# apcamargo/genomad

Measured on NVIDIA H100. Metric: nn_classification_windows_per_s, higher is better.
Workload: dtype split operands on wgmma (conv: fp16 main pass + two e4m3 correction passes; w_v: 3 fp16 passes), fp32 accumulate; fp32-equivalent (<=1e-4 vs the fp32 oracle, measured ~1e-5)

## Files before the change

### genomad_b200/csrc/api.cu

```cuda
#include <cuda.h>
#include <cuda_runtime.h>
#include <cuda_fp16.h>

#include <algorithm>
#include <cmath>
#include <cstdio>
#include <cstring>
#include <string>
#include <vector>

#include "../../include/gnm.h"
#include "common.cuh"
#include "encode.cuh"
#include "conv_t.cuh"
#include "layer1_wv.cuh"
#include "conv_ref.cuh"
#include "igloo.cuh"
#include "dense.cuh"
#include "logits_tc.cuh"
#include "wv_gather.cuh"

using namespace gnm;

static thread_local std::string g_err;
static int fail(const std::string& m) { g_err = m; return 1; }

#define GNM_CUDA(expr)                                                                       \
  do {                                                                                       \
    cudaError_t e__ = (expr);                                                                \
    if (e__ != cudaSuccess)                                                                  \
      return fail(std::string(#expr) + " failed: " + cudaGetErrorString(e__) + " (" __FILE__ \
                  ":" + std::to_string(__LINE__) + ")");                                     \
  } while (0)

extern "C" const char* gnm_last_error(void) { return g_err.c_str(); }
extern "C" const char* gnm_version(void) { return "libgnm 0.4 (sm_90a; wgmma fp16 + e4m3 split convs, fused fp16x3 w_v + patch gather, tf32x3 logits and dense head)"; }

struct StageTimer {
  std::vector<const char*> names;
  std::vector<cudaEvent_t> events;
};

struct gnm_handle {
  int device = 0;
  int max_batch = 0;
  int num_sms = 0;
  long long launches = 0;
  int conv_impl = 0;
  int debug_stop = 0;
  int profile_stages = 0;
  int conv_experiment = 0;
  int conv_cluster = 1;
  int fuse_gather = 1;
  int fuse_l1 = 0;
  long long* conv_dbg = nullptr;
  float* conv1_table = nullptr; float* conv1_triple = nullptr; float* conv1_bias = nullptr;
  uint8_t* wpack[4] = {nullptr, nullptr, nullptr, nullptr};
  float conv_out_scale[2] = {1.f, 1.f};
  float* conv_bias[2] = {nullptr, nullptr};
  float* conv_w32[2] = {nullptr, nullptr};
  float* wv32[2] = {nullptr, nullptr};
  float* ent_w[2] = {nullptr, nullptr}; int32_t* ent_pos[2] = {nullptr, nullptr}; int32_t* slot_of[2] = {nullptr, nullptr};
  float* wbias[2] = {nullptr, nullptr}; float* wqk[2] = {nullptr, nullptr};
  float* d0w = nullptr; float* d0b = nullptr; float* bn0_scale = nullptr; float* bn0_shift = nullptr;
  float* d1w = nullptr; float* d1b = nullptr; float* bn1_scale = nullptr; float* bn1_shift = nullptr;
  float* d2w = nullptr; float* d2b = nullptr;
  float* dwT_hi[2] = {nullptr, nullptr}; float* dwT_lo[2] = {nullptr, nullptr};
  float* hA_hi[2] = {nullptr, nullptr}; float* hA_lo[2] = {nullptr, nullptr};
  CUtensorMap tm_hd_a[2][2]; CUtensorMap tm_hd_b[2][2];
  uint8_t* ybuf[2] = {nullptr, nullptr};
  int ybuf_fp8lo[2] = {0, 0};
  float* q[2] = {nullptr, nullptr};
  float* mpi[2] = {nullptr, nullptr};
  float* mpi_hi[2] = {nullptr, nullptr}; float* mpi_lo[2] = {nullptr, nullptr};
  float* wqkT_hi[2] = {nullptr, nullptr}; float* wqkT_lo[2] = {nullptr, nullptr};
  CUtensorMap tm_lg_a[2][2];
  CUtensorMap tm_lg_b[2][2];
  float* part = nullptr;
  int2* grp[2] = {nullptr, nullptr};
  int32_t* band_gstart[2] = {nullptr, nullptr};
  uint4* wfrag[2] = {nullptr, nullptr};
  float gather_unscale[2] = {1.f, 1.f};
  float wv_out_scale[2] = {1.f, 1.f};
  std::vector<int32_t> band_groups[2];
  int32_t* cta_split = nullptr;
  std::vector<int32_t> split_host[2];
  int split_groups[2] = {-1, -1}, split_grid[2] = {-1, -1};
  float wv_cost_base = 1.f, wv_cost_group = 0.1f;
  int mb_pad = 0;
  CUtensorMap tm_band[2];
  float* logits = nullptr; float* logits_part = nullptr; float* h0 = nullptr; float* h1 = nullptr; float* h2 = nullptr;
  float* scratch32 = nullptr;
  uint8_t* in_stage[2] = {nullptr, nullptr};
  float* out_stage[2] = {nullptr, nullptr};
  float* q_set[2][2] = {{nullptr, nullptr}, {nullptr, nullptr}};
  float* mpi_set[2][2] = {{nullptr, nullptr}, {nullptr, nullptr}};
  float* mpi_hi_set[2][2] = {{nullptr, nullptr}, {nullptr, nullptr}};
  float* mpi_lo_set[2][2] = {{nullptr, nullptr}, {nullptr, nullptr}};
  CUtensorMap tm_lg_a_set[2][2][2];
  int tail_overlap = 1;
  cudaStream_t tail_stream = nullptr;
  cudaEvent_t main_done[2] = {nullptr, nullptr}, tail_done[2] = {nullptr, nullptr};
  cudaStream_t copy_stream = nullptr, compute_stream = nullptr;
  cudaEvent_t in_ready[2] = {nullptr, nullptr}, in_free[2] = {nullptr, nullptr};
  DeviceStatus* status = nullptr;
  CUtensorMap tm_act[2];
  CUtensorMap tm_w[4];
  CUtensorMap tm_w_half[4];
  StageTimer timer;
  std::vector<void*> allocs;
};

template <class T>
static int dev_upload(gnm_handle* h, T** dst, const T* src, size_t count) {
  GNM_CUDA(cudaMalloc(reinterpret_cast<void**>(dst), count * sizeof(T)));
  h->allocs.push_back(*dst);
  GNM_CUDA(cudaMemcpy(*dst, src, count * sizeof(T), cudaMemcpyHostToDevice));
  return 0;
}
template <class T>
static int dev_alloc(gnm_handle* h, T** dst, size_t count) {
  GNM_CUDA(cudaMalloc(reinterpret_cast<void**>(dst), count * sizeof(T)));
  h->allocs.push_back(*dst);
  return 0;
}

typedef CUresult (*PFN_encodeTiled)(CUtensorMap*, CUtensorMapDataType, cuuint32_t, void*, const cuuint64_t*,
                                    const cuuint64_t*, const cuuint32_t*, const cuuint32_t*, CUtensorMapInterleave,
                                    CUtensorMapSwizzle, CUtensorMapL2promotion, CUtensorMapFloatOOBfill);

static int get_encode_fn(PFN_encodeTiled* fn) {
  void* p = nullptr;
  cudaDriverEntryPointQueryResult qres;
  GNM_CUDA(cudaGetDriverEntryPoint("cuTensorMapEncodeTiled", &p, cudaEnableDefault, &qres));
  if (qres != cudaDriverEntryPointSuccess || !p) return fail("cuTensorMapEncodeTiled not available from the driver");
  *fn = reinterpret_cast<PFN_encodeTiled>(p);
  return 0;
}

static int make_act_map(PFN_encodeTiled enc, CUtensorMap* tm, uint8_t* base, int n_windows, int box_rows = kSlabRows) {
  cuuint64_t dims[3] = {kRowBytes, kTok, static_cast<cuuint64_t>(n_windows)};
  cuuint64_t strides[2] = {kRowBytes, static_cast<cuuint64_t>(kTok) * kRowBytes};
  cuuint32_t box[3] = {128, static_cast<cuuint32_t>(box_rows), 1};
  cuuint32_t estr[3] = {1, 1, 1};
  CUresult r = enc(tm, CU_TENSOR_MAP_DATA_TYPE_UINT8, 3, base, dims, strides, box, estr,
                   CU_TENSOR_MAP_INTERLEAVE_NONE, CU_TENSOR_MAP_SWIZZLE_128B, CU_TENSOR_MAP_L2_PROMOTION_L2_128B,
                   CU_TENSOR_MAP_FLOAT_OOB_FILL_NONE);
  if (r != CUDA_SUCCESS) return fail("cuTensorMapEncodeTiled(activations) failed: " + std::to_string(int(r)));
  return 0;
}
static int make_band_map(PFN_encodeTiled enc, CUtensorMap* tm, uint8_t* base, int n_windows) {
  cuuint64_t dims[3] = {kRowBytes, static_cast<cuuint64_t>(n_windows), kTok};
  cuuint64_t strides[2] = {static_cast<cuuint64_t>(kTok) * kRowBytes, kRowBytes};
  cuuint32_t box[3] = {128, kBandWins, kBandRows};
  cuuint32_t estr[3] = {1, 1, 1};
  CUresult r = enc(tm, CU_TENSOR_MAP_DATA_TYPE_UINT8, 3, base, dims, strides, box, estr,
                   CU_TENSOR_MAP_INTERLEAVE_NONE, CU_TENSOR_MAP_SWIZZLE_128B, CU_TENSOR_MAP_L2_PROMOTION_L2_128B,
                   CU_TENSOR_MAP_FLOAT_OOB_FILL_NONE);
  if (r != CUDA_SUCCESS) return fail("cuTensorMapEncodeTiled(activation bands) failed: " + std::to_string(int(r)));
  return 0;
}
static int make_w_map(PFN_encodeTiled enc, CUtensorMap* tm, uint8_t* base, int n_stages, int box_rows) {
  cuuint64_t dims[2] = {128, static_cast<cuuint64_t>(n_stages) * 128};
  cuuint64_t strides[1] = {128};
  cuuint32_t box[2] = {128, static_cast<cuuint32_t>(box_rows)};
  cuuint32_t estr[2] = {1, 1};
  CUresult r = enc(tm, CU_TENSOR_MAP_DATA_TYPE_UINT8, 2, base, dims, strides, box, estr,
                   CU_TENSOR_MAP_INTERLEAVE_NONE, CU_TENSOR_MAP_SWIZZLE_128B, CU_TENSOR_MAP_L2_PROMOTION_L2_256B,
                   CU_TENSOR_MAP_FLOAT_OOB_FILL_NONE);
  if (r != CUDA_SUCCESS) return fail("cuTensorMapEncodeTiled(weights) failed: " + std::to_string(int(r)));
  return 0;
}

static int make_f32_map(PFN_encodeTiled enc, CUtensorMap* tm, float* base, int inner, int rows, int box_rows) {
  cuuint64_t dims[2] = {static_cast<cuuint64_t>(inner), static_cast<cuuint64_t>(rows)};
  cuuint64_t strides[1] = {static_cast<cuuint64_t>(inner) * sizeof(float)};
  cuuint32_t box[2] = {32, static_cast<cuuint32_t>(box_rows)};
  cuuint32_t estr[2] = {1, 1};
  CUresult r = enc(tm, CU_TENSOR_MAP_DATA_TYPE_FLOAT32, 2, base, dims, strides, box, estr,
                   CU_TENSOR_MAP_INTERLEAVE_NONE, CU_TENSOR_MAP_SWIZZLE_128B, CU_TENSOR_MAP_L2_PROMOTION_L2_256B,
                   CU_TENSOR_MAP_FLOAT_OOB_FILL_NONE);
  if (r != CUDA_SUCCESS) return fail("cuTensorMapEncodeTiled(fp32 matrix) failed: " + std::to_string(int(r)));
  return 0;
}

static void pack_stage_f16(std::vector<uint8_t>& dst, const float* Wkn , int w_lo, int kh, float scale) {
  for (int n = 0; n < kC; ++n)
    for (int kk = 0; kk < 64; ++kk) {
      const float x = Wkn[static_cast<size_t>(kh * 64 + kk) * kC + n] * scale;
      const __half hi = __float2half_rn(x);
      const float v = w_lo ? x - __half2float(hi) : __half2float(hi);
      const uint16_t bits = __half_as_ushort(__float2half_rn(v));
      dst.push_back(static_cast<uint8_t>(bits & 0xff));
      dst.push_back(static_cast<uint8_t>(bits >> 8));
    }
}
static void pack_stage_f8_pairs(std::vector<uint8_t>& dst, const float* Wkn, int kh, float scale, float scale_hi, float scale_lo) {
  for (int n = 0; n < kC; ++n)
    for (int c = 0; c < 64; ++c) {
      const float x = Wkn[static_cast<size_t>(kh * 64 + c) * kC + n] * scale;
      const float hi = __half2float(__float2half_rn(x));
      dst.push_back(static_cast<uint8_t>(__nv_cvt_float_to_fp8(hi * scale_hi, __NV_SATFINITE, __NV_E4M3)));
      dst.push_back(static_cast<uint8_t>(__nv_cvt_float_to_fp8((x - hi) * scale_lo, __NV_SATFINITE, __NV_E4M3)));
    }
}

struct PatchPack {
  std::vector<float> ent_w;
  std::vector<int32_t> ent_pos, slot_of;
  std::vector<int2> groups;
  std::vector<int32_t> band_gstart;
  std::vector<uint32_t> frag;
  float unscale = 1.f;
};
static void pack_patches(const int32_t* patches, const float* w_mult, const float* w_summer, PatchPack& o) {
  std::vector<int> order(static_cast<size_t>(kPatches) * kPatchLen);
  for (size_t i = 0; i < order.size(); ++i) order[i] = static_cast<int>(i);
  std::stable_sort(order.begin(), order.end(), [&](int a, int b) { return patches[a] < patches[b]; });
  o.ent_w.assign(static_cast<size_t>(kGsSlots) * kC, 0.f);
  o.ent_pos.assign(kGsSlots, 0);
  o.slot_of.assign(static_cast<size_t>(kPatches) * kPatchLen, 0);
  std::vector<float>& ent_w = o.ent_w;
  std::vector<int32_t>& ent_pos = o.ent_pos;
  for (size_t slot = 0; slot < order.size(); ++slot) {
    const int e = order[slot], k = e % kPatchLen;
    ent_pos[slot] = patches[e];
    o.slot_of[e] = static_cast<int32_t>(slot);
    for (int c = 0; c < kC; ++c)
      ent_w[slot * kC + c] = (w_mult[static_cast<size_t>(e) * kC + c] * w_summer[k * kC + c]) * (1.f / kActScale);
  }
  float wmax = 0.f;
  for (float v : ent_w) wmax = std::max(wmax, std::fabs(v));
  int k2 = 0;
  if (wmax > 0.f && std::isfinite(wmax)) { int ex; std::frexp(wmax, &ex); k2 = std::max(-24, std::min(40, 14 - ex)); }
  const float wscale = std::ldexp(1.f, k2);
  o.unscale = std::ldexp(1.f, -k2);
  o.groups.clear();
  o.band_gstart.assign(kNumBands + 1, 0);
  const size_t n_ent = order.size();
  size_t slot = 0;
  for (int b = 0; b < kNumBands; ++b) {
    o.band_gstart[b] = static_cast<int32_t>(o.groups.size());
    while (slot < n_ent && ent_pos[slot] < (b + 1) * kBandRows) {
      size_t run = slot;
      while (run < n_ent && ent_pos[run] == ent_pos[slot] && run - slot < static_cast<size_t>(kWgGroupMax)) ++run;
      o.groups.push_back(make_int2(static_cast<int>(slot), (ent_pos[slot] - b * kBandRows) | (static_cast<int>(run - slot) << 8)));
      slot = run;
    }
  }
  o.band_gstart[kNumBands] = static_cast<int32_t>(o.groups.size());
  if (o.groups.empty()) o.groups.push_back(make_int2(0, 0));
  auto h2 = [](float x, float y) {
    return static_cast<uint32_t>(__half_as_ushort(__float2half_rn(x))) | (static_cast<uint32_t>(__half_as_ushort(__float2half_rn(y))) << 16);
  };
  o.frag.assign(static_cast<size_t>(kGsSlots) * 128, 0u);
  for (size_t e = 0; e < n_ent; ++e)
    for (int kh = 0; kh < 2; ++kh)
      for (int ks = 0; ks < 4; ++ks)
        for (int tig = 0; tig < 4; ++tig) {
          const int k0 = kh * 64 + ks * 16 + 2 * tig;
          const int kk[4] = {k0, k0 + 1, k0 + 8, k0 + 9};
          float hi[4], lo[4];
          for (int i = 0; i < 4; ++i) {
            const float x = ent_w[e * kC + kk[i]] * wscale;
            hi[i] = __half2float(__float2half_rn(x));
            lo[i] = x - hi[i];
          }
          uint32_t* f = &o.frag[(((e * 2 + kh) * 4 + ks) * 4 + tig) * 4];
          f[0] = h2(hi[0], hi[1]); f[1] = h2(hi[2], hi[3]); f[2] = h2(lo[0], lo[1]); f[3] = h2(lo[2], lo[3]);
        }
}
extern "C" int gnm_pack_patches(const int32_t* patches, const float* w_mult, const float* w_summer, int32_t* slot_of, int32_t* ent_pos,
                                float* ent_w, int32_t* groups, int* n_groups, int32_t* band_first_group, uint32_t* frag, float* unscale,
                                int* layout) {
  if (layout) { layout[0] = kBandRows; layout[1] = kNumBands; layout[2] = kGsSlots; layout[3] = kWgGroupMax; }
  if (!patches && !w_mult && !w_summer) return 0;
  if (!patches || !w_mult || !w_summer || !n_groups) return fail("gnm_pack_patches: null argument");
  for (int i = 0; i < kPatches * kPatchLen; ++i)
    if (patches[i] < 0 || patches[i] >= kTok) return fail("gnm_pack_patches: patch index out of range");
  PatchPack pk;
  pack_patches(patches, w_mult, w_summer, pk);
  const int real_groups = pk.band_gstart[kNumBands];
  if (groups && *n_groups < real_groups) return fail("gnm_pack_patches: groups buffer too small");
  if (slot_of) std::memcpy(slot_of, pk.slot_of.data(), pk.slot_of.size() * sizeof(int32_t));
  if (ent_pos) std::memcpy(ent_pos, pk.ent_pos.data(), pk.ent_pos.size() * sizeof(int32_t));
  if (ent_w) std::memcpy(ent_w, pk.ent_w.data(), pk.ent_w.size() * sizeof(float));
  if (groups) for (int i = 0; i < real_groups; ++i) { groups[2 * i] = pk.groups[i].x; groups[2 * i + 1] = pk.groups[i].y; }
  *n_groups = real_groups;
  if (band_first_group) std::memcpy(band_first_group, pk.band_gstart.data(), pk.band_gstart.size() * sizeof(int32_t));
  if (frag) std::memcpy(frag, pk.frag.data(), pk.frag.size() * sizeof(uint32_t));
  if (unscale) *unscale = pk.unscale;
  return 0;
}

extern "C" int gnm_create(int device, const gnm_weights* w, int max_batch, gnm_handle** out) {
  if (!w || !out) return fail("gnm_create: null argument");
  if (max_batch < 1 || max_batch > 32768) return fail("gnm_create: max_batch must be in [1, 32768]");
  int ndev = 0;
  if (cudaGetDeviceCount(&ndev) != cudaSuccess || ndev == 0)
    return fail("gnm_create: no CUDA device available (libgnm has no CPU fallback)");
  if (device < 0 || device >= ndev) return fail("gnm_create: bad device index");
  cudaDeviceProp prop;
  GNM_CUDA(cudaGetDeviceProperties(&prop, device));
  if (prop.major != 9 || prop.minor != 0)
    return fail(std::string("gnm_create: device is sm_") + std::to_string(prop.major * 10 + prop.minor) +
                ", this library is built for sm_90a (H100) only");
  GNM_CUDA(cudaSetDevice(device));
// ... 764 lines not shown
```

### genomad_b200/csrc/wv_gather.cuh

```cuda
#pragma once
#include <cuda.h>
#include <type_traits>
#include "common.cuh"
#include "conv_t.cuh"
#include "igloo.cuh"

namespace gnm {

constexpr int kBandRows   = 24;
constexpr int kBandWins   = 8;
constexpr int kWgN        = kBandRows * kBandWins;
constexpr int kNumBands   = (kTok + kBandRows - 1) / kBandRows;
constexpr int kWgRegion   = kWgN * 128;
constexpr int kWgBufs     = 6;
constexpr int kWgSlab     = kWgBufs * kWgRegion;
constexpr int kWgWBytes   = kWvStages * kBStage;
constexpr int kWgMmaWarps = 8;
constexpr int kWgWarps    = 15;
constexpr int kWgThreads  = (kWgMmaWarps + kWgWarps + 1) * 32;
constexpr int kWgGroupCap = 2;
constexpr int kWgGroupMax = 4;
constexpr int kWgSmem     = kWgSlab + kWgWBytes + 2048;
static_assert(kWgSmem <= 232448, "wv_gather_kernel exceeds the 227 KB of shared memory a CTA may use");
static_assert(kWgN == 3 * 64 && kBandRows == 3 * kPool && kBandWins == 8, "unit shape: three pool groups of 8 positions x 8 windows");
static_assert(kWgRegion % 1024 == 0, "regions must keep the 1024-byte alignment of the 128-byte swizzle");

struct WvGatherParams {
  float* q_out;
  float out_scale;
  const int2* grp;
  const int32_t* band_gstart;
  const uint4* wfrag;
  float gather_unscale;
  float* part_t;
  int n_windows, n_pad;
  int groups;
  int n_units;
  const int32_t* cta_split;
  int experiment;
  long long* dbg;
  DeviceStatus* status;
};

__device__ __forceinline__ uint2 ldg_frag(const uint2* p) {
  uint2 v;
  asm volatile("ld.global.nc.L1::evict_last.v2.u32 {%0, %1}, [%2];" : "=r"(v.x), "=r"(v.y) : "l"(p));
  return v;
}
__device__ __forceinline__ void ldsm_x4(uint32_t saddr, uint32_t (&a)[4]) {
  asm volatile("ldmatrix.sync.aligned.m8n8.x4.shared.b16 {%0, %1, %2, %3}, [%4];"
               : "=r"(a[0]), "=r"(a[1]), "=r"(a[2]), "=r"(a[3]) : "r"(saddr));
}
__device__ __forceinline__ void mma_16816(float (&d)[4], const uint32_t (&a)[4], uint32_t b0, uint32_t b1) {
  asm volatile("mma.sync.aligned.m16n8k16.row.col.f32.f16.f16.f32 {%0, %1, %2, %3}, {%4, %5, %6, %7}, {%8, %9}, {%0, %1, %2, %3};"
               : "+f"(d[0]), "+f"(d[1]), "+f"(d[2]), "+f"(d[3]) : "r"(a[0]), "r"(a[1]), "r"(a[2]), "r"(a[3]), "r"(b0), "r"(b1));
}

__global__ void __launch_bounds__(kWgThreads, 1)
wv_gather_kernel(const __grid_constant__ CUtensorMap tm_band, const __grid_constant__ CUtensorMap tm_w, const WvGatherParams p) {
  extern __shared__ uint8_t smem_raw[];
  uint8_t* smem = reinterpret_cast<uint8_t*>((reinterpret_cast<uintptr_t>(smem_raw) + 1023) & ~uintptr_t(1023));
  uint8_t* s_a = smem;
  uint8_t* s_w = smem + kWgSlab;
  uint64_t* bars = reinterpret_cast<uint64_t*>(s_w + kWgWBytes);
  uint64_t* a_full = bars;
  uint64_t* a_empty = bars + 8;
  uint64_t* w_full = bars + 16;

  const int warp = threadIdx.x >> 5, lane = threadIdx.x & 31;
  constexpr int kProducerWarp = kWgMmaWarps + kWgWarps;
  const int u_begin = p.cta_split[blockIdx.x], u_end = p.cta_split[blockIdx.x + 1];

  if (warp == kProducerWarp && lane == 0) {
    tma_prefetch_desc(&tm_band);
    tma_prefetch_desc(&tm_w);
    for (int i = 0; i < kWgBufs; ++i) { mbar_init(&a_full[i], 1); mbar_init(&a_empty[i], kWgMmaWarps + kWgWarps); }
    mbar_init(w_full, 1);
    fence_barrier_init();
  }
  __syncthreads();

  if (warp == kProducerWarp && lane == 0) {
    mbar_arrive_expect_tx(w_full, kWgWBytes);
    for (int q = 0; q < kWvStages; ++q) tma_load_2d_hint(s_w + q * kBStage, &tm_w, w_full, 0, q * 128, l2_policy_evict_last());
    const uint64_t pol = l2_policy_evict_first();
    uint32_t phases = 0;
    int b0 = 0;
    for (int unit = u_begin; unit < u_end; ++unit) {
      const int band = unit / p.groups;
      const int w0 = (unit - band * p.groups) * kBandWins;
#pragma unroll
      for (int k = 0; k < 4; ++k) {
        int b = b0 + k; if (b >= kWgBufs) b -= kWgBufs;
        mbar_wait(&a_empty[b], ((phases >> b) & 1) ^ 1, p.status, 500 + b);
        phases ^= 1u << b;
        mbar_arrive_expect_tx(&a_full[b], kWgRegion);
        const int src = (k & 1 ? kOffLo16 : kOffHi16) + (k >> 1) * 128;
        tma_load_3d_hint(s_a + b * kWgRegion, &tm_band, &a_full[b], src, w0, band * kBandRows, pol);
      }
      b0 += 4; if (b0 >= kWgBufs) b0 -= kWgBufs;
    }
  } else if (warp < kWgMmaWarps) {
    const int g = warp >> 2, wq = warp & 3;
    const uint32_t a_base = smem_u32(s_a);
    const uint32_t w_base = smem_u32(s_w) + g * 64 * 128;
    const int ch0 = g * 64 + wq * 16 + (lane >> 2);
    const int win0 = 2 * (lane & 3);
    const float oscale = p.out_scale;
    mbar_wait(w_full, 0, p.status, 510);
    uint32_t phases = 0;
    int b0 = 0;
    float d[32];
    for (int unit = u_begin; unit < u_end; ++unit) {
      const int band = unit / p.groups;
      const int w0 = (unit - band * p.groups) * kBandWins;
      int bufs[4];
#pragma unroll
      for (int k = 0; k < 4; ++k) {
        int b = b0 + k; if (b >= kWgBufs) b -= kWgBufs;
        bufs[k] = b;
        mbar_wait(&a_full[b], (phases >> b) & 1, p.status, 530 + b);
        phases ^= 1u << b;
      }
#pragma unroll 1
      for (int pg = 0; pg < kBandRows / kPool; ++pg) {
        wgmma_fence();
#pragma unroll 1
        for (int kh = 0; kh < 2; ++kh) {
          const uint64_t yh = gmma_desc_sw128(a_base + bufs[2 * kh] * kWgRegion + pg * 64 * 128);
          const uint64_t yl = gmma_desc_sw128(a_base + bufs[2 * kh + 1] * kWgRegion + pg * 64 * 128);
          const uint64_t whi = gmma_desc_sw128(w_base + (2 * kh) * kBStage);
          const uint64_t wlo = gmma_desc_sw128(w_base + (2 * kh + 1) * kBStage);
#pragma unroll
          for (int kk = 0; kk < 4; ++kk) {
            wgmma_f16_n64(d, whi + kk * 2, yh + kk * 2, (kh == 0 && kk == 0) ? 0u : 1u);
            wgmma_f16_n64(d, whi + kk * 2, yl + kk * 2, 1u);
          }
#pragma unroll
          for (int kk = 0; kk < 4; ++kk) wgmma_f16_n64(d, wlo + kk * 2, yh + kk * 2, 1u);
        }
        wgmma_commit();
        wgmma_wait<0>();
        wgmma_fence_regs(d);
        const int gg = band * (kBandRows / kPool) + pg;
        if (gg < kPooled && !(p.experiment & 128)) {
#pragma unroll
          for (int h = 0; h < 2; ++h)
#pragma unroll
            for (int e = 0; e < 2; ++e) {
              float m = d[2 * h + e];
#pragma unroll
              for (int i = 1; i < kPool; ++i) m = fmaxf(m, d[4 * i + 2 * h + e]);
              const int w = w0 + win0 + e;
              if (w < p.n_windows) p.q_out[(static_cast<size_t>(w) * kPooled + gg) * kC + ch0 + 8 * h] = m * oscale;
            }
        }
      }
      __syncwarp();
      if (lane == 0)
#pragma unroll
        for (int k = 0; k < 4; ++k) mbar_arrive(&a_empty[bufs[k]]);
      b0 += 4; if (b0 >= kWgBufs) b0 -= kWgBufs;
    }
  } else if (warp >= kWgMmaWarps && warp < kWgMmaWarps + kWgWarps) {
    const int gw = warp - kWgMmaWarps;
    const float gscale = p.gather_unscale;
    const int lm_plane = (lane >> 3) & 1, lm_chunk = lane >> 4, lm_win = lane & 7;
    const int gid = lane >> 2, tig = lane & 3;
    const uint32_t slab = smem_u32(s_a);
    int it = 0;
    uint32_t phases = 0;
    int b0 = 0;
    long long c_wait_full = 0, c_gather = 0, tq = 0;
    const long long t_begin = clock64();
    int cur_band = -1, g_first = 0, g_cnt = 0, n_mine = 0;
    int my_e0[kWgGroupCap] = {0, 0}, my_meta[kWgGroupCap] = {0, 0};
    bool fast = true;
    auto gather_group = [&](int e0, int meta, int kh, uint32_t hi_base, uint32_t lo_base) -> float {
      const int row = meta & 31, ne = meta >> 8;
      const uint2* wf = reinterpret_cast<const uint2*>(p.wfrag) + ((static_cast<size_t>(e0 + (gid >> 1)) * 2 + kh) * 16 + tig) * 2 + (gid & 1);
      uint2 b[4];
#pragma unroll
      for (int ks = 0; ks < 4; ++ks) b[ks] = ((gid >> 1) < ne && !(p.experiment & 1024)) ? ldg_frag(wf + ks * 8) : make_uint2(0u, 0u);
      const uint32_t rb = (lm_plane ? lo_base : hi_base) + row * (kBandWins * 128) + lm_win * 128;
      uint32_t a[4][4];
#pragma unroll
      for (int ks = 0; ks < 4; ++ks) {
        if (p.experiment & 2048) { a[ks][0] = a[ks][1] = a[ks][2] = a[ks][3] = rb; continue; }
        ldsm_x4(rb + (((ks * 2 + lm_chunk) ^ lm_win) << 4), a[ks]);
      }
      float d[4][4];
#pragma unroll
      for (int ks = 0; ks < 4; ++ks) d[ks][0] = d[ks][1] = d[ks][2] = d[ks][3] = 0.f;
      if (p.experiment & 256) {
#pragma unroll
        for (int ks = 0; ks < 4; ++ks) asm volatile("" :: "r"(a[ks][0] | a[ks][1] | a[ks][2] | a[ks][3] | b[ks].x | b[ks].y));
      } else {
#pragma unroll
        for (int ks = 0; ks < 4; ++ks) mma_16816(d[ks], a[ks], b[ks].x, b[ks].y);
      }
      float v = 0.f;
#pragma unroll
      for (int ks = 0; ks < 4; ++ks) v += (d[ks][0] + d[ks][2]) + (d[ks][1] + d[ks][3]);
      return v * gscale;
    };
    for (int unit = u_begin; unit < u_end; ++unit, ++it) {
      const int band = unit / p.groups;
      const int w0 = (unit - band * p.groups) * kBandWins;
      if (band != cur_band) {
        cur_band = band;
        g_first = p.band_gstart[band];
        g_cnt = (p.experiment & 32) ? 0 : p.band_gstart[band + 1] - g_first;
        fast = g_cnt <= kWgWarps * kWgGroupCap;
        n_mine = 0;
#pragma unroll
        for (int i = 0; i < kWgGroupCap; ++i) {
          const int gi = gw + i * kWgWarps;
          if (fast && gi < g_cnt) { const int2 m = p.grp[g_first + gi]; my_e0[i] = m.x; my_meta[i] = m.y; n_mine = i + 1; }
        }
      }
      float c0[kWgGroupCap];
#pragma unroll 1
      for (int kh = 0; kh < 2; ++kh) {
        int bh = b0 + 2 * kh; if (bh >= kWgBufs) bh -= kWgBufs;
        int bl = b0 + 2 * kh + 1; if (bl >= kWgBufs) bl -= kWgBufs;
        const uint32_t ph_h = (phases >> bh) & 1, ph_l = (phases >> bl) & 1;
        phases ^= (1u << bh) | (1u << bl);
        const uint32_t hi_base = slab + bh * kWgRegion, lo_base = slab + bl * kWgRegion;
        if (p.dbg) tq = clock64();
        mbar_wait(&a_full[bh], ph_h, p.status, 550 + bh);
        mbar_wait(&a_full[bl], ph_l, p.status, 560 + bl);
        if (p.dbg) { const long long t = clock64(); c_wait_full += t - tq; tq = t; }
        if (fast) {
#pragma unroll
          for (int i = 0; i < kWgGroupCap; ++i)
            if (i < n_mine) {
              const float v = gather_group(my_e0[i], my_meta[i], kh, hi_base, lo_base);
              if (kh == 0) c0[i] = v;
              else if (tig < (my_meta[i] >> 8) && !(p.experiment & 64))
                p.part_t[static_cast<size_t>(my_e0[i] + tig) * p.n_pad + w0 + gid] = c0[i] + v;
            }
        } else {
#pragma unroll 1
          for (int gi = gw; gi < g_cnt; gi += kWgWarps) {
            const int2 m = p.grp[g_first + gi];
            const float v = gather_group(m.x, m.y, kh, hi_base, lo_base);
            if (tig < (m.y >> 8)) {
              float* gp = p.part_t + static_cast<size_t>(m.x + tig) * p.n_pad + w0 + gid;
              *gp = kh == 0 ? v : *gp + v;
            }
          }
        }
        __syncwarp();
        if (lane == 0) { mbar_arrive(&a_empty[bh]); mbar_arrive(&a_empty[bl]); }
        if (p.dbg) c_gather += clock64() - tq;
      }
      b0 += 4; if (b0 >= kWgBufs) b0 -= kWgBufs;
    }
    if (p.dbg && warp == kWgMmaWarps && lane == 0) {
      long long* d = p.dbg + blockIdx.x * 8;
      d[0] = clock64() - t_begin; d[1] = c_wait_full; d[2] = c_gather; d[5] = it;
    }
  }
}

__global__ void __launch_bounds__(256)
patch_finish_t_kernel(const float* __restrict__ part_t, const int32_t* __restrict__ slot_of, const float* __restrict__ w_bias,
                      float* __restrict__ mpi, float* __restrict__ mpi_hi, float* __restrict__ mpi_lo, int n_windows, int n_pad) {
  __shared__ float tile[32][33];
  const int p0 = blockIdx.x * 32, w0 = blockIdx.y * 32;
  const int tx = threadIdx.x & 31, ty = threadIdx.x >> 5;
  for (int pp = ty; pp < 32; pp += 8) {
    const int pch = p0 + pp, w = w0 + tx;
    float v = 0.f;
    if (pch < kPatches && w < n_windows) {
      const int4 s4 = *reinterpret_cast<const int4*>(slot_of + pch * 4);
      v = (((part_t[static_cast<size_t>(s4.x) * n_pad + w] + part_t[static_cast<size_t>(s4.y) * n_pad + w]) +
            part_t[static_cast<size_t>(s4.z) * n_pad + w]) + part_t[static_cast<size_t>(s4.w) * n_pad + w]) + w_bias[pch];
    }
    tile[pp][tx] = v;
  }
  __syncthreads();
  for (int ww = ty; ww < 32; ww += 8) {
    const int pch = p0 + tx, w = w0 + ww;
    if (pch < kPatches && w < n_windows) {
      const float v = tile[tx][ww];
      const size_t o = static_cast<size_t>(w) * kPatches + pch;
      mpi[o] = v;
      const float hi = __uint_as_float(__float_as_uint(v) & 0xffffe000u);
      mpi_hi[o] = hi;
      mpi_lo[o] = __uint_as_float(__float_as_uint(v - hi) & 0xffffe000u);
    }
  }
}

}
```

Before: 74440.

## Pipeline w_v gather at pool-group granularity with an 18-slot TMA box ring

Replaces the six band-sized shared buffers with an 18-slot ring of smaller boxes, one box per pool group, plane and half. The producer now issues four boxes per pool group, and consumers release slots after each pool group instead of after a whole band. The goal is to shorten the pipeline stall between units and keep the wgmma and gather warps fed with a deeper prefetch. Gather warps now process both k-halves of a group together and skip groups outside the current pool group. The cost is more TMA issues and barrier traffic, plus always-on clock64 timing in the MMA warps.

```diff
diff --git a/genomad_b200/csrc/api.cu b/genomad_b200/csrc/api.cu
--- a/genomad_b200/csrc/api.cu
+++ b/genomad_b200/csrc/api.cu
@@ -152,7 +152,7 @@
 static int make_band_map(PFN_encodeTiled enc, CUtensorMap* tm, uint8_t* base, int n_windows) {
   cuuint64_t dims[3] = {kRowBytes, static_cast<cuuint64_t>(n_windows), kTok};
   cuuint64_t strides[2] = {static_cast<cuuint64_t>(kTok) * kRowBytes, kRowBytes};
-  cuuint32_t box[3] = {128, kBandWins, kBandRows};
+  cuuint32_t box[3] = {128, kBandWins, kPool};
   cuuint32_t estr[3] = {1, 1, 1};
   CUresult r = enc(tm, CU_TENSOR_MAP_DATA_TYPE_UINT8, 3, base, dims, strides, box, estr,
                    CU_TENSOR_MAP_INTERLEAVE_NONE, CU_TENSOR_MAP_SWIZZLE_128B, CU_TENSOR_MAP_L2_PROMOTION_L2_128B,
diff --git a/genomad_b200/csrc/wv_gather.cuh b/genomad_b200/csrc/wv_gather.cuh
--- a/genomad_b200/csrc/wv_gather.cuh
+++ b/genomad_b200/csrc/wv_gather.cuh
@@ -11,9 +11,10 @@
 constexpr int kBandWins   = 8;
 constexpr int kWgN        = kBandRows * kBandWins;
 constexpr int kNumBands   = (kTok + kBandRows - 1) / kBandRows;
-constexpr int kWgRegion   = kWgN * 128;
-constexpr int kWgBufs     = 6;
-constexpr int kWgSlab     = kWgBufs * kWgRegion;
+constexpr int kWgBox      = kPool * kBandWins * 128;
+constexpr int kWgBoxes    = 4 * (kBandRows / kPool);
+constexpr int kWgSlots    = 18;
+constexpr int kWgSlab     = kWgSlots * kWgBox;
 constexpr int kWgWBytes   = kWvStages * kBStage;
 constexpr int kWgMmaWarps = 8;
 constexpr int kWgWarps    = 15;
@@ -23,7 +24,8 @@
 constexpr int kWgSmem     = kWgSlab + kWgWBytes + 2048;
 static_assert(kWgSmem <= 232448, "wv_gather_kernel exceeds the 227 KB of shared memory a CTA may use");
 static_assert(kWgN == 3 * 64 && kBandRows == 3 * kPool && kBandWins == 8, "unit shape: three pool groups of 8 positions x 8 windows");
-static_assert(kWgRegion % 1024 == 0, "regions must keep the 1024-byte alignment of the 128-byte swizzle");
+static_assert(kWgBox % 1024 == 0, "boxes must keep the 1024-byte alignment of the 128-byte swizzle");
+static_assert(kWgSlots >= 4, "every consumer holds one pool group's four boxes at a time");
 
 struct WvGatherParams {
   float* q_out;
@@ -56,6 +58,9 @@
                : "+f"(d[0]), "+f"(d[1]), "+f"(d[2]), "+f"(d[3]) : "r"(a[0]), "r"(a[1]), "r"(a[2]), "r"(a[3]), "r"(b0), "r"(b1));
 }
 
+__device__ __forceinline__ uint32_t wg_slot(uint32_t L) { return L % kWgSlots; }
+__device__ __forceinline__ uint32_t wg_parity(uint32_t L) { return (L / kWgSlots) & 1; }
+
 __global__ void __launch_bounds__(kWgThreads, 1)
 wv_gather_kernel(const __grid_constant__ CUtensorMap tm_band, const __grid_constant__ CUtensorMap tm_w, const WvGatherParams p) {
   extern __shared__ uint8_t smem_raw[];
@@ -64,41 +69,44 @@
   uint8_t* s_w = smem + kWgSlab;
   uint64_t* bars = reinterpret_cast<uint64_t*>(s_w + kWgWBytes);
   uint64_t* a_full = bars;
-  uint64_t* a_empty = bars + 8;
-  uint64_t* w_full = bars + 16;
-
-  const int warp = threadIdx.x >> 5, lane = threadIdx.x & 31;
+  uint64_t* a_empty = bars + kWgSlots;
+  uint64_t* w_full = bars + 2 * kWgSlots;
+
+  const int warp = __shfl_sync(0xffffffffu, static_cast<int>(threadIdx.x) >> 5, 0);
+  const int lane = threadIdx.x & 31;
   constexpr int kProducerWarp = kWgMmaWarps + kWgWarps;
   const int u_begin = p.cta_split[blockIdx.x], u_end = p.cta_split[blockIdx.x + 1];
 
-  if (warp == kProducerWarp && lane == 0) {
-    tma_prefetch_desc(&tm_band);
-    tma_prefetch_desc(&tm_w);
-    for (int i = 0; i < kWgBufs; ++i) { mbar_init(&a_full[i], 1); mbar_init(&a_empty[i], kWgMmaWarps + kWgWarps); }
-    mbar_init(w_full, 1);
-    fence_barrier_init();
+  if (warp == kProducerWarp) {
+    if (elect_one()) {
+      tma_prefetch_desc(&tm_band);
+      tma_prefetch_desc(&tm_w);
+      for (int i = 0; i < kWgSlots; ++i) { mbar_init(&a_full[i], 1); mbar_init(&a_empty[i], kWgMmaWarps + kWgWarps); }
+      mbar_init(w_full, 1);
+      fence_barrier_init();
+    }
   }
   __syncthreads();
 
-  if (warp == kProducerWarp && lane == 0) {
-    mbar_arrive_expect_tx(w_full, kWgWBytes);
-    for (int q = 0; q < kWvStages; ++q) tma_load_2d_hint(s_w + q * kBStage, &tm_w, w_full, 0, q * 128, l2_policy_evict_last());
-    const uint64_t pol = l2_policy_evict_first();
-    uint32_t phases = 0;
-    int b0 = 0;
-    for (int unit = u_begin; unit < u_end; ++unit) {
-      const int band = unit / p.groups;
-      const int w0 = (unit - band * p.groups) * kBandWins;
-#pragma unroll
-      for (int k = 0; k < 4; ++k) {
-        int b = b0 + k; if (b >= kWgBufs) b -= kWgBufs;
-        mbar_wait(&a_empty[b], ((phases >> b) & 1) ^ 1, p.status, 500 + b);
-        phases ^= 1u << b;
-        mbar_arrive_expect_tx(&a_full[b], kWgRegion);
-        const int src = (k & 1 ? kOffLo16 : kOffHi16) + (k >> 1) * 128;
-        tma_load_3d_hint(s_a + b * kWgRegion, &tm_band, &a_full[b], src, w0, band * kBandRows, pol);
-      }
-      b0 += 4; if (b0 >= kWgBufs) b0 -= kWgBufs;
+  if (warp == kProducerWarp) {
+    if (elect_one()) {
+      mbar_arrive_expect_tx(w_full, kWgWBytes);
+      for (int q = 0; q < kWvStages; ++q) tma_load_2d_hint(s_w + q * kBStage, &tm_w, w_full, 0, q * 128, l2_policy_evict_last());
+      const uint64_t pol = l2_policy_evict_first();
+      uint32_t L = 0;
+      for (int unit = u_begin; unit < u_end; ++unit) {
+        const int band = unit / p.groups;
+        const int w0 = (unit - band * p.groups) * kBandWins;
+        for (int pg = 0; pg < kBandRows / kPool; ++pg)
+#pragma unroll
+          for (int r = 0; r < 4; ++r, ++L) {
+            const uint32_t s = wg_slot(L);
+            mbar_wait(&a_empty[s], wg_parity(L) ^ 1, p.status, 500 + s);
+            mbar_arrive_expect_tx(&a_full[s], kWgBox);
+            const int src = (r & 1 ? kOffLo16 : kOffHi16) + (r >> 1) * 128;
+            tma_load_3d_hint(s_a + s * kWgBox, &tm_band, &a_full[s], src, w0, band * kBandRows + pg * kPool, pol);
+          }
+      }
     }
   } else if (warp < kWgMmaWarps) {
     const int g = warp >> 2, wq = warp & 3;
@@ -108,27 +116,28 @@
     const int win0 = 2 * (lane & 3);
     const float oscale = p.out_scale;
     mbar_wait(w_full, 0, p.status, 510);
-    uint32_t phases = 0;
-    int b0 = 0;
+    long long c_wait = 0, c_mma = 0, c_epi = 0;
+    uint32_t L = 0;
     float d[32];
     for (int unit = u_begin; unit < u_end; ++unit) {
       const int band = unit / p.groups;
       const int w0 = (unit - band * p.groups) * kBandWins;
-      int bufs[4];
-#pragma unroll
-      for (int k = 0; k < 4; ++k) {
-        int b = b0 + k; if (b >= kWgBufs) b -= kWgBufs;
-        bufs[k] = b;
-        mbar_wait(&a_full[b], (phases >> b) & 1, p.status, 530 + b);
-        phases ^= 1u << b;
-      }
 #pragma unroll 1
-      for (int pg = 0; pg < kBandRows / kPool; ++pg) {
+      for (int pg = 0; pg < kBandRows / kPool; ++pg, L += 4) {
+        uint32_t s[4];
+        long long tq = clock64();
+#pragma unroll
+        for (int r = 0; r < 4; ++r) {
+          s[r] = wg_slot(L + r);
+          mbar_wait(&a_full[s[r]], wg_parity(L + r), p.status, 530 + r);
+        }
+        long long t = clock64();
+        c_wait += t - tq; tq = t;
         wgmma_fence();
-#pragma unroll 1
+#pragma unroll
         for (int kh = 0; kh < 2; ++kh) {
-          const uint64_t yh = gmma_desc_sw128(a_base + bufs[2 * kh] * kWgRegion + pg * 64 * 128);
-          const uint64_t yl = gmma_desc_sw128(a_base + bufs[2 * kh + 1] * kWgRegion + pg * 64 * 128);
+          const uint64_t yh = gmma_desc_sw128(a_base + s[2 * kh] * kWgBox);
+          const uint64_t yl = gmma_desc_sw128(a_base + s[2 * kh + 1] * kWgBox);
           const uint64_t whi = gmma_desc_sw128(w_base + (2 * kh) * kBStage);
           const uint64_t wlo = gmma_desc_sw128(w_base + (2 * kh + 1) * kBStage);
 #pragma unroll
@@ -142,6 +151,12 @@
         wgmma_commit();
         wgmma_wait<0>();
         wgmma_fence_regs(d);
+        t = clock64();
+        c_mma += t - tq; tq = t;
+        __syncwarp();
+        if (lane == 0)
+#pragma unroll
+          for (int r = 0; r < 4; ++r) mbar_arrive(&a_empty[s[r]]);
         const int gg = band * (kBandRows / kPool) + pg;
         if (gg < kPooled && !(p.experiment & 128)) {
 #pragma unroll
@@ -155,34 +170,33 @@
               if (w < p.n_windows) p.q_out[(static_cast<size_t>(w) * kPooled + gg) * kC + ch0 + 8 * h] = m * oscale;
             }
         }
-      }
-      __syncwarp();
-      if (lane == 0)
-#pragma unroll
-        for (int k = 0; k < 4; ++k) mbar_arrive(&a_empty[bufs[k]]);
-      b0 += 4; if (b0 >= kWgBufs) b0 -= kWgBufs;
-    }
-  } else if (warp >= kWgMmaWarps && warp < kWgMmaWarps + kWgWarps) {
+        c_epi += clock64() - tq;
+      }
+    }
+    if (p.dbg && wq == 0 && lane == 0) {
+      long long* dd = p.dbg + blockIdx.x * 8;
+      if (g == 0) { dd[3] = c_wait; dd[4] = c_mma; dd[6] = c_epi; }
+      else dd[7] = c_mma;
+    }
+  } else {
     const int gw = warp - kWgMmaWarps;
     const float gscale = p.gather_unscale;
     const int lm_plane = (lane >> 3) & 1, lm_chunk = lane >> 4, lm_win = lane & 7;
     const int gid = lane >> 2, tig = lane & 3;
     const uint32_t slab = smem_u32(s_a);
     int it = 0;
-    uint32_t phases = 0;
-    int b0 = 0;
     long long c_wait_full = 0, c_gather = 0, tq = 0;
     const long long t_begin = clock64();
     int cur_band = -1, g_first = 0, g_cnt = 0, n_mine = 0;
     int my_e0[kWgGroupCap] = {0, 0}, my_meta[kWgGroupCap] = {0, 0};
     bool fast = true;
-    auto gather_group = [&](int e0, int meta, int kh, uint32_t hi_base, uint32_t lo_base) -> float {
+    auto gather_group = [&](int e0, int meta, int kh, uint32_t Lp) -> float {
       const int row = meta & 31, ne = meta >> 8;
       const uint2* wf = reinterpret_cast<const uint2*>(p.wfrag) + ((static_cast<size_t>(e0 + (gid >> 1)) * 2 + kh) * 16 + tig) * 2 + (gid & 1);
       uint2 b[4];
 #pragma unroll
       for (int ks = 0; ks < 4; ++ks) b[ks] = ((gid >> 1) < ne && !(p.experiment & 1024)) ? ldg_frag(wf + ks * 8) : make_uint2(0u, 0u);
-      const uint32_t rb = (lm_plane ? lo_base : hi_base) + row * (kBandWins * 128) + lm_win * 128;
+      const uint32_t rb = slab + wg_slot(Lp) * kWgBox + (row & 7) * (kBandWins * 128) + lm_win * 128;
       uint32_t a[4][4];
 #pragma unroll
       for (int ks = 0; ks < 4; ++ks) {
@@ -219,43 +233,39 @@
           if (fast && gi < g_cnt) { const int2 m = p.grp[g_first + gi]; my_e0[i] = m.x; my_meta[i] = m.y; n_mine = i + 1; }
         }
       }
-      float c0[kWgGroupCap];
 #pragma unroll 1
-      for (int kh = 0; kh < 2; ++kh) {
-        int bh = b0 + 2 * kh; if (bh >= kWgBufs) bh -= kWgBufs;
-        int bl = b0 + 2 * kh + 1; if (bl >= kWgBufs) bl -= kWgBufs;
-        const uint32_t ph_h = (phases >> bh) & 1, ph_l = (phases >> bl) & 1;
-        phases ^= (1u << bh) | (1u << bl);
-        const uint32_t hi_base = slab + bh * kWgRegion, lo_base = slab + bl * kWgRegion;
+      for (int pg = 0; pg < kBandRows / kPool; ++pg) {
+        const uint32_t Lg = static_cast<uint32_t>(kWgBoxes * it + 4 * pg);
         if (p.dbg) tq = clock64();
-        mbar_wait(&a_full[bh], ph_h, p.status, 550 + bh);
-        mbar_wait(&a_full[bl], ph_l, p.status, 560 + bl);
+#pragma unroll
+        for (int r = 0; r < 4; ++r) mbar_wait(&a_full[wg_slot(Lg + r)], wg_parity(Lg + r), p.status, 550 + r);
+        const uint32_t Lp = Lg + lm_plane;
         if (p.dbg) { const long long t = clock64(); c_wait_full += t - tq; tq = t; }
         if (fast) {
 #pragma unroll
           for (int i = 0; i < kWgGroupCap; ++i)
-            if (i < n_mine) {
-              const float v = gather_group(my_e0[i], my_meta[i], kh, hi_base, lo_base);
-              if (kh == 0) c0[i] = v;
-              else if (tig < (my_meta[i] >> 8) && !(p.experiment & 64))
-                p.part_t[static_cast<size_t>(my_e0[i] + tig) * p.n_pad + w0 + gid] = c0[i] + v;
+            if (i < n_mine && ((my_meta[i] & 31) >> 3) == pg) {
+              const float c0 = gather_group(my_e0[i], my_meta[i], 0, Lp);
+              const float v = gather_group(my_e0[i], my_meta[i], 1, Lp + 2);
+              if (tig < (my_meta[i] >> 8) && !(p.experiment & 64))
+                p.part_t[static_cast<size_t>(my_e0[i] + tig) * p.n_pad + w0 + gid] = c0 + v;
             }
         } else {
 #pragma unroll 1
           for (int gi = gw; gi < g_cnt; gi += kWgWarps) {
             const int2 m = p.grp[g_first + gi];
-            const float v = gather_group(m.x, m.y, kh, hi_base, lo_base);
-            if (tig < (m.y >> 8)) {
-              float* gp = p.part_t + static_cast<size_t>(m.x + tig) * p.n_pad + w0 + gid;
-              *gp = kh == 0 ? v : *gp + v;
-            }
+            if (((m.y & 31) >> 3) != pg) continue;
+            const float c0 = gather_group(m.x, m.y, 0, Lp);
+            const float v = gather_group(m.x, m.y, 1, Lp + 2);
+            if (tig < (m.y >> 8)) p.part_t[static_cast<size_t>(m.x + tig) * p.n_pad + w0 + gid] = c0 + v;
           }
         }
         __syncwarp();
-        if (lane == 0) { mbar_arrive(&a_empty[bh]); mbar_arrive(&a_empty[bl]); }
+        if (lane == 0)
+#pragma unroll
+          for (int r = 0; r < 4; ++r) mbar_arrive(&a_empty[wg_slot(Lg + r)]);
         if (p.dbg) c_gather += clock64() - tq;
       }
-      b0 += 4; if (b0 >= kWgBufs) b0 -= kWgBufs;
     }
     if (p.dbg && warp == kWgMmaWarps && lane == 0) {
       long long* d = p.dbg + blockIdx.x * 8;
```

After: 76270, median of 6. +2.5%, better.

## Split w_v gather band loads into per-pool-group slots with finer pipelining

Applied to the files above, without the earlier changes.

The TMA band loads shrink from whole 24-row bands to 8-row pool-group slots, using an 18-slot ring in place of 6 region buffers. The MMA warps and gather warps now wait on and release each pool group's four slots separately. This lets the producer refill buffers sooner and lets consumers start on the first pool group before the whole band has landed, so load latency overlaps more with compute. The cost is more TMA issues and mbarrier operations per unit, plus one loop pass per pool group in the gather warps that filters groups by their pool index. The change also adds clock64 debug counters to the MMA warps, which only run when a debug buffer is supplied.

```diff
diff --git a/genomad_b200/csrc/api.cu b/genomad_b200/csrc/api.cu
--- a/genomad_b200/csrc/api.cu
+++ b/genomad_b200/csrc/api.cu
@@ -152,7 +152,7 @@
 static int make_band_map(PFN_encodeTiled enc, CUtensorMap* tm, uint8_t* base, int n_windows) {
   cuuint64_t dims[3] = {kRowBytes, static_cast<cuuint64_t>(n_windows), kTok};
   cuuint64_t strides[2] = {static_cast<cuuint64_t>(kTok) * kRowBytes, kRowBytes};
-  cuuint32_t box[3] = {128, kBandWins, kBandRows};
+  cuuint32_t box[3] = {128, kBandWins, kPool};
   cuuint32_t estr[3] = {1, 1, 1};
   CUresult r = enc(tm, CU_TENSOR_MAP_DATA_TYPE_UINT8, 3, base, dims, strides, box, estr,
                    CU_TENSOR_MAP_INTERLEAVE_NONE, CU_TENSOR_MAP_SWIZZLE_128B, CU_TENSOR_MAP_L2_PROMOTION_L2_128B,
diff --git a/genomad_b200/csrc/wv_gather.cuh b/genomad_b200/csrc/wv_gather.cuh
--- a/genomad_b200/csrc/wv_gather.cuh
+++ b/genomad_b200/csrc/wv_gather.cuh
@@ -11,9 +11,10 @@
 constexpr int kBandWins   = 8;
 constexpr int kWgN        = kBandRows * kBandWins;
 constexpr int kNumBands   = (kTok + kBandRows - 1) / kBandRows;
-constexpr int kWgRegion   = kWgN * 128;
-constexpr int kWgBufs     = 6;
-constexpr int kWgSlab     = kWgBufs * kWgRegion;
+constexpr int kWgSlot     = kPool * kBandWins * 128;
+constexpr int kWgSlotsU   = 12;
+constexpr int kWgSlots    = 18;
+constexpr int kWgSlab     = kWgSlots * kWgSlot;
 constexpr int kWgWBytes   = kWvStages * kBStage;
 constexpr int kWgMmaWarps = 8;
 constexpr int kWgWarps    = 15;
@@ -23,7 +24,7 @@
 constexpr int kWgSmem     = kWgSlab + kWgWBytes + 2048;
 static_assert(kWgSmem <= 232448, "wv_gather_kernel exceeds the 227 KB of shared memory a CTA may use");
 static_assert(kWgN == 3 * 64 && kBandRows == 3 * kPool && kBandWins == 8, "unit shape: three pool groups of 8 positions x 8 windows");
-static_assert(kWgRegion % 1024 == 0, "regions must keep the 1024-byte alignment of the 128-byte swizzle");
+static_assert(kWgSlot % 1024 == 0, "slots must keep the 1024-byte alignment of the 128-byte swizzle");
 
 struct WvGatherParams {
   float* q_out;
@@ -64,41 +65,39 @@
   uint8_t* s_w = smem + kWgSlab;
   uint64_t* bars = reinterpret_cast<uint64_t*>(s_w + kWgWBytes);
   uint64_t* a_full = bars;
-  uint64_t* a_empty = bars + 8;
-  uint64_t* w_full = bars + 16;
-
-  const int warp = threadIdx.x >> 5, lane = threadIdx.x & 31;
+  uint64_t* a_empty = bars + kWgSlots;
+  uint64_t* w_full = bars + 2 * kWgSlots;
+
+  const int warp = __shfl_sync(0xffffffffu, static_cast<int>(threadIdx.x) >> 5, 0);
+  const int lane = threadIdx.x & 31;
   constexpr int kProducerWarp = kWgMmaWarps + kWgWarps;
   const int u_begin = p.cta_split[blockIdx.x], u_end = p.cta_split[blockIdx.x + 1];
 
-  if (warp == kProducerWarp && lane == 0) {
+  if (threadIdx.x == kProducerWarp * 32) {
     tma_prefetch_desc(&tm_band);
     tma_prefetch_desc(&tm_w);
-    for (int i = 0; i < kWgBufs; ++i) { mbar_init(&a_full[i], 1); mbar_init(&a_empty[i], kWgMmaWarps + kWgWarps); }
+    for (int i = 0; i < kWgSlots; ++i) { mbar_init(&a_full[i], 1); mbar_init(&a_empty[i], kWgMmaWarps + kWgWarps); }
     mbar_init(w_full, 1);
     fence_barrier_init();
   }
   __syncthreads();
 
-  if (warp == kProducerWarp && lane == 0) {
+  if (warp == kProducerWarp && elect_one()) {
     mbar_arrive_expect_tx(w_full, kWgWBytes);
     for (int q = 0; q < kWvStages; ++q) tma_load_2d_hint(s_w + q * kBStage, &tm_w, w_full, 0, q * 128, l2_policy_evict_last());
     const uint64_t pol = l2_policy_evict_first();
-    uint32_t phases = 0;
-    int b0 = 0;
+    uint32_t ld = 0;
     for (int unit = u_begin; unit < u_end; ++unit) {
       const int band = unit / p.groups;
       const int w0 = (unit - band * p.groups) * kBandWins;
-#pragma unroll
-      for (int k = 0; k < 4; ++k) {
-        int b = b0 + k; if (b >= kWgBufs) b -= kWgBufs;
-        mbar_wait(&a_empty[b], ((phases >> b) & 1) ^ 1, p.status, 500 + b);
-        phases ^= 1u << b;
-        mbar_arrive_expect_tx(&a_full[b], kWgRegion);
-        const int src = (k & 1 ? kOffLo16 : kOffHi16) + (k >> 1) * 128;
-        tma_load_3d_hint(s_a + b * kWgRegion, &tm_band, &a_full[b], src, w0, band * kBandRows, pol);
-      }
-      b0 += 4; if (b0 >= kWgBufs) b0 -= kWgBufs;
+#pragma unroll 1
+      for (int k = 0; k < kWgSlotsU; ++k, ++ld) {
+        const int s = ld % kWgSlots;
+        mbar_wait(&a_empty[s], ((ld / kWgSlots) & 1) ^ 1, p.status, 500 + s);
+        mbar_arrive_expect_tx(&a_full[s], kWgSlot);
+        const int src = (k & 1 ? kOffLo16 : kOffHi16) + ((k >> 1) & 1) * 128;
+        tma_load_3d_hint(s_a + s * kWgSlot, &tm_band, &a_full[s], src, w0, band * kBandRows + (k >> 2) * kPool, pol);
+      }
     }
   } else if (warp < kWgMmaWarps) {
     const int g = warp >> 2, wq = warp & 3;
@@ -107,28 +106,29 @@
     const int ch0 = g * 64 + wq * 16 + (lane >> 2);
     const int win0 = 2 * (lane & 3);
     const float oscale = p.out_scale;
-    mbar_wait(w_full, 0, p.status, 510);
-    uint32_t phases = 0;
-    int b0 = 0;
+    mbar_wait(w_full, 0, p.status, 520);
+    uint32_t ld = 0;
+    long long c_wait_full = 0, c_mma = 0, c_epi = 0, tq = 0;
+    const long long t_begin = clock64();
     float d[32];
     for (int unit = u_begin; unit < u_end; ++unit) {
       const int band = unit / p.groups;
       const int w0 = (unit - band * p.groups) * kBandWins;
-      int bufs[4];
-#pragma unroll
-      for (int k = 0; k < 4; ++k) {
-        int b = b0 + k; if (b >= kWgBufs) b -= kWgBufs;
-        bufs[k] = b;
-        mbar_wait(&a_full[b], (phases >> b) & 1, p.status, 530 + b);
-        phases ^= 1u << b;
-      }
 #pragma unroll 1
-      for (int pg = 0; pg < kBandRows / kPool; ++pg) {
+      for (int pg = 0; pg < kBandRows / kPool; ++pg, ld += 4) {
+        int s[4];
+        if (p.dbg) tq = clock64();
+#pragma unroll
+        for (int k = 0; k < 4; ++k) {
+          s[k] = (ld + k) % kWgSlots;
+          mbar_wait(&a_full[s[k]], ((ld + k) / kWgSlots) & 1, p.status, 530 + s[k]);
+        }
+        if (p.dbg) { const long long t = clock64(); c_wait_full += t - tq; tq = t; }
         wgmma_fence();
-#pragma unroll 1
+#pragma unroll
         for (int kh = 0; kh < 2; ++kh) {
-          const uint64_t yh = gmma_desc_sw128(a_base + bufs[2 * kh] * kWgRegion + pg * 64 * 128);
-          const uint64_t yl = gmma_desc_sw128(a_base + bufs[2 * kh + 1] * kWgRegion + pg * 64 * 128);
+          const uint64_t yh = gmma_desc_sw128(a_base + s[2 * kh] * kWgSlot);
+          const uint64_t yl = gmma_desc_sw128(a_base + s[2 * kh + 1] * kWgSlot);
           const uint64_t whi = gmma_desc_sw128(w_base + (2 * kh) * kBStage);
           const uint64_t wlo = gmma_desc_sw128(w_base + (2 * kh + 1) * kBStage);
 #pragma unroll
@@ -142,6 +142,11 @@
         wgmma_commit();
         wgmma_wait<0>();
         wgmma_fence_regs(d);
+        __syncwarp();
+        if (lane == 0)
+#pragma unroll
+          for (int k = 0; k < 4; ++k) mbar_arrive(&a_empty[s[k]]);
+        if (p.dbg) { const long long t = clock64(); c_mma += t - tq; tq = t; }
         const int gg = band * (kBandRows / kPool) + pg;
         if (gg < kPooled && !(p.experiment & 128)) {
 #pragma unroll
@@ -155,12 +160,12 @@
               if (w < p.n_windows) p.q_out[(static_cast<size_t>(w) * kPooled + gg) * kC + ch0 + 8 * h] = m * oscale;
             }
         }
-      }
-      __syncwarp();
-      if (lane == 0)
-#pragma unroll
-        for (int k = 0; k < 4; ++k) mbar_arrive(&a_empty[bufs[k]]);
-      b0 += 4; if (b0 >= kWgBufs) b0 -= kWgBufs;
+        if (p.dbg) c_epi += clock64() - tq;
+      }
+    }
+    if (p.dbg && warp == 0 && lane == 0) {
+      long long* dd = p.dbg + blockIdx.x * 8;
+      dd[3] = c_wait_full; dd[4] = c_mma; dd[6] = c_epi; dd[7] = clock64() - t_begin;
     }
   } else if (warp >= kWgMmaWarps && warp < kWgMmaWarps + kWgWarps) {
     const int gw = warp - kWgMmaWarps;
@@ -169,15 +174,14 @@
     const int gid = lane >> 2, tig = lane & 3;
     const uint32_t slab = smem_u32(s_a);
     int it = 0;
-    uint32_t phases = 0;
-    int b0 = 0;
+    uint32_t ld = 0;
     long long c_wait_full = 0, c_gather = 0, tq = 0;
     const long long t_begin = clock64();
     int cur_band = -1, g_first = 0, g_cnt = 0, n_mine = 0;
     int my_e0[kWgGroupCap] = {0, 0}, my_meta[kWgGroupCap] = {0, 0};
     bool fast = true;
     auto gather_group = [&](int e0, int meta, int kh, uint32_t hi_base, uint32_t lo_base) -> float {
-      const int row = meta & 31, ne = meta >> 8;
+      const int row = meta & 7, ne = meta >> 8;
       const uint2* wf = reinterpret_cast<const uint2*>(p.wfrag) + ((static_cast<size_t>(e0 + (gid >> 1)) * 2 + kh) * 16 + tig) * 2 + (gid & 1);
       uint2 b[4];
 #pragma unroll
@@ -221,41 +225,41 @@
       }
       float c0[kWgGroupCap];
 #pragma unroll 1
-      for (int kh = 0; kh < 2; ++kh) {
-        int bh = b0 + 2 * kh; if (bh >= kWgBufs) bh -= kWgBufs;
-        int bl = b0 + 2 * kh + 1; if (bl >= kWgBufs) bl -= kWgBufs;
-        const uint32_t ph_h = (phases >> bh) & 1, ph_l = (phases >> bl) & 1;
-        phases ^= (1u << bh) | (1u << bl);
-        const uint32_t hi_base = slab + bh * kWgRegion, lo_base = slab + bl * kWgRegion;
-        if (p.dbg) tq = clock64();
-        mbar_wait(&a_full[bh], ph_h, p.status, 550 + bh);
-        mbar_wait(&a_full[bl], ph_l, p.status, 560 + bl);
-        if (p.dbg) { const long long t = clock64(); c_wait_full += t - tq; tq = t; }
-        if (fast) {
-#pragma unroll
-          for (int i = 0; i < kWgGroupCap; ++i)
-            if (i < n_mine) {
-              const float v = gather_group(my_e0[i], my_meta[i], kh, hi_base, lo_base);
-              if (kh == 0) c0[i] = v;
-              else if (tig < (my_meta[i] >> 8) && !(p.experiment & 64))
-                p.part_t[static_cast<size_t>(my_e0[i] + tig) * p.n_pad + w0 + gid] = c0[i] + v;
-            }
-        } else {
+      for (int pg = 0; pg < kBandRows / kPool; ++pg) {
+#pragma unroll
+        for (int kh = 0; kh < 2; ++kh, ld += 2) {
+          const int sh = ld % kWgSlots, sl = (ld + 1) % kWgSlots;
+          const uint32_t hi_base = slab + sh * kWgSlot, lo_base = slab + sl * kWgSlot;
+          if (p.dbg) tq = clock64();
+          mbar_wait(&a_full[sh], (ld / kWgSlots) & 1, p.status, 550 + sh);
+          mbar_wait(&a_full[sl], ((ld + 1) / kWgSlots) & 1, p.status, 570 + sl);
+          if (p.dbg) { const long long t = clock64(); c_wait_full += t - tq; tq = t; }
+          if (fast) {
+#pragma unroll
+            for (int i = 0; i < kWgGroupCap; ++i)
+              if (i < n_mine && ((my_meta[i] & 31) >> 3) == pg) {
+                const float v = gather_group(my_e0[i], my_meta[i], kh, hi_base, lo_base);
+                if (kh == 0) c0[i] = v;
+                else if (tig < (my_meta[i] >> 8) && !(p.experiment & 64))
+                  p.part_t[static_cast<size_t>(my_e0[i] + tig) * p.n_pad + w0 + gid] = c0[i] + v;
+              }
+          } else {
 #pragma unroll 1
-          for (int gi = gw; gi < g_cnt; gi += kWgWarps) {
-            const int2 m = p.grp[g_first + gi];
-            const float v = gather_group(m.x, m.y, kh, hi_base, lo_base);
-            if (tig < (m.y >> 8)) {
-              float* gp = p.part_t + static_cast<size_t>(m.x + tig) * p.n_pad + w0 + gid;
-              *gp = kh == 0 ? v : *gp + v;
+            for (int gi = gw; gi < g_cnt; gi += kWgWarps) {
+              const int2 m = p.grp[g_first + gi];
+              if (((m.y & 31) >> 3) != pg) continue;
+              const float v = gather_group(m.x, m.y, kh, hi_base, lo_base);
+              if (tig < (m.y >> 8)) {
+                float* gp = p.part_t + static_cast<size_t>(m.x + tig) * p.n_pad + w0 + gid;
+                *gp = kh == 0 ? v : *gp + v;
+              }
             }
           }
-        }
-        __syncwarp();
-        if (lane == 0) { mbar_arrive(&a_empty[bh]); mbar_arrive(&a_empty[bl]); }
-        if (p.dbg) c_gather += clock64() - tq;
-      }
-      b0 += 4; if (b0 >= kWgBufs) b0 -= kWgBufs;
+          __syncwarp();
+          if (lane == 0) { mbar_arrive(&a_empty[sh]); mbar_arrive(&a_empty[sl]); }
+          if (p.dbg) c_gather += clock64() - tq;
+        }
+      }
     }
     if (p.dbg && warp == kWgMmaWarps && lane == 0) {
       long long* d = p.dbg + blockIdx.x * 8;
```

New measurement: 73770 before, 74960 after, median of 6. +1.6%, better.
